# chernistry/sentio

Measured on NVIDIA B200. Metric: retrieval queries/sec @1M docs,1024-d,top_k=100, higher is better.
Workload: dtype f16 store / f32 scan / f64 exact re-score

## Files before the change

### sentio_b200/csrc/api.cu

```cuda
#include <stdarg.h>
#include <stdlib.h>

#include "common.cuh"

static thread_local char g_err[1024] = "";

void sb_set_error(const char* fmt, ...) {
  va_list ap;
  va_start(ap, fmt);
  vsnprintf(g_err, sizeof(g_err), fmt, ap);
  va_end(ap);
}

void ce_model_free(CeModel* m);
void ce_tokens_free(CeDocTokens* t);
void bm25_build_free(Bm25Build* b);

extern "C" {

const char* sb_last_error(void) { return g_err; }

int sb_version(void) { return 1000; }

int sb_create(int device, sb_ctx** out) {
  SB_REQUIRE(out != nullptr, SB_ERR_ARG, "sb_create: out is NULL");
  *out = nullptr;
  int ndev = 0;
  cudaError_t e = cudaGetDeviceCount(&ndev);
  if (e != cudaSuccess || ndev == 0) {
    sb_set_error("sb_create: no CUDA device visible (%s); libsentio_b200 has no CPU fallback",
                 e != cudaSuccess ? cudaGetErrorString(e) : "device count is 0");
    return SB_ERR_CUDA;
  }
  SB_REQUIRE(device >= 0 && device < ndev, SB_ERR_ARG, "sb_create: device %d out of range [0,%d)", device, ndev);
  DeviceGuard g(device);
  cudaDeviceProp prop;
  SB_CUDA(cudaGetDeviceProperties(&prop, device));
  SB_REQUIRE(prop.major == 10, SB_ERR_UNSUPPORTED,
             "sb_create: device %d is sm_%d%d; this library is built for sm_100a (B200) only", device, prop.major,
             prop.minor);
  sb_ctx* ctx = new sb_ctx();
  ctx->device = device;
  ctx->num_sms = prop.multiProcessorCount;
  ctx->smem_optin = prop.sharedMemPerBlockOptin;
  if (const char* v = getenv("SB_DENSE_PAIR")) ctx->dense_pair = atoi(v) != 0;
  if (const char* v = getenv("SB_DENSE_SAMPLE")) ctx->dense_sample_per_cta = atoi(v) > 0 ? atoi(v) : 2;
  if (const char* v = getenv("SB_DENSE_MULTISAMPLE")) ctx->dense_multisample = atoi(v) != 0;
  if (const char* v = getenv("SB_DENSE_PREFETCH")) ctx->dense_prefetch = atoi(v) > 0 ? atoi(v) : 0;
  if (const char* v = getenv("SB_DENSE_STAGES")) ctx->dense_max_stages = atoi(v) >= 3 ? atoi(v) : 8;
  cudaError_t se = cudaStreamCreateWithFlags(&ctx->stream, cudaStreamNonBlocking);
  if (se != cudaSuccess) {
    sb_set_error("sb_create: cudaStreamCreate failed: %s", cudaGetErrorString(se));
    delete ctx;
    return SB_ERR_CUDA;
  }
  *out = ctx;
  return SB_OK;
}

void sb_destroy(sb_ctx* ctx) {
  if (!ctx) return;
  DeviceGuard g(ctx->device);
  cudaStreamSynchronize(ctx->stream);
  for (int s = 0; s < SB_MAX_DENSE_SLOTS; ++s) {
    if (ctx->dense[s].rows) cudaFree(ctx->dense[s].rows);
    if (ctx->dense[s].inv_norm) cudaFree(ctx->dense[s].inv_norm);
  }
  Bm25Index& b = ctx->bm25;
  if (b.indptr) cudaFree(b.indptr);
  if (b.post_doc) cudaFree(b.post_doc);
  if (b.post_ratio) cudaFree(b.post_ratio);
  if (b.dnorm) cudaFree(b.dnorm);
  if (b.idf) cudaFree(b.idf);
  if (b.dense_of_term) cudaFree(b.dense_of_term);
  if (b.dense_ratio) cudaFree(b.dense_ratio);
  if (ctx->ce) ce_model_free(ctx->ce);
  if (ctx->enc) ce_model_free(ctx->enc);
  if (ctx->ce_tokens) ce_tokens_free(ctx->ce_tokens);
  if (ctx->bm25_build) bm25_build_free(ctx->bm25_build);
  ctx->q_dev.release();
  ctx->cand_dev.release();
  ctx->out_ids_dev.release();
  ctx->out_sc_dev.release();
  ctx->out_cnt_dev.release();
  ctx->misc_dev.release();
  ctx->misc2_dev.release();
  ctx->misc3_dev.release();
  ctx->acc_dev.release();
  ctx->qn_dev.release();
  ctx->qaux_dev.release();
  ctx->doc_chars_dev.release();
  ctx->pin_in.release();
  ctx->pin_out.release();
  ctx->hyb_pin.release();
  ctx->hyb_dev.release();
  for (auto& r : ctx->prof_recs) { cudaEventDestroy(r.a); cudaEventDestroy(r.b); }
  for (auto e : ctx->prof_pool) cudaEventDestroy(e);
  cudaStreamDestroy(ctx->stream);
// ... 67 lines not shown
```

### sentio_b200/csrc/common.cuh

```cuda
#pragma once
#include <cuda_runtime.h>
#include <cuda_fp16.h>
#include <stdint.h>
#include <stdio.h>
#include <mutex>
#include <string>
#include <vector>

#include "../../include/sentio_b200.h"

void sb_set_error(const char* fmt, ...);

#define SB_CUDA(expr)                                                                         \
  do {                                                                                        \
    cudaError_t _e = (expr);                                                                  \
    if (_e != cudaSuccess) {                                                                  \
      sb_set_error("CUDA error %s at %s:%d: %s", cudaGetErrorName(_e), __FILE__, __LINE__,    \
                   cudaGetErrorString(_e));                                                   \
      return SB_ERR_CUDA;                                                                     \
    }                                                                                         \
  } while (0)

#define SB_REQUIRE(cond, code, ...)  \
  do {                               \
// ... 51 lines not shown
    p = nullptr;
    cap = 0;
  }
  template <typename T>
  T* as() const { return reinterpret_cast<T*>(p); }
};

struct DenseIndex {
  int64_t n = 0;
  int64_t n_pad = 0;
  int32_t d = 0;
  int32_t d_pad = 0;
  int64_t id_base = 0;
  __half* rows = nullptr;
  float* inv_norm = nullptr;
  alignas(64) unsigned char tm_rows[128] = {0};
  const void* tm_rows_ptr = nullptr;
};

struct Bm25Index {
  int64_t n_docs = 0, n_terms = 0, nnz = 0;
  int64_t id_base = 0;
  int32_t variant = 0;
  double k1 = 1.5, b = 0.75, delta = 1.0, avgdl = 0.0;
  int64_t* indptr = nullptr;
  int32_t* post_doc = nullptr;
  double* post_ratio = nullptr;
  double* dnorm = nullptr;
  double* idf = nullptr;
  int32_t n_dense = 0;
  int32_t* dense_of_term = nullptr;
  double* dense_ratio = nullptr;
};

struct CeModel;
struct CeDocTokens;
struct Bm25Build;

struct sb_ctx {
  int device = 0;
  int num_sms = 0;
  size_t smem_optin = 0;
  cudaStream_t stream = nullptr;
  std::mutex mu;
  DenseIndex dense[SB_MAX_DENSE_SLOTS];
  Bm25Index bm25;
  CeModel* ce = nullptr;
  CeModel* enc = nullptr;
  CeDocTokens* ce_tokens = nullptr;
  Bm25Build* bm25_build = nullptr;
  int dense_mode = 0;
  int dense_pair = 1;
  int dense_sample_per_cta = 2;
  int max_clusters2 = 0;
  int dense_multisample = 1;
  int dense_prefetch = 0;
  int dense_max_stages = 8;
  uint64_t launches = 0;
  bool prof_on = false;
  struct ProfRec { int id; cudaEvent_t a, b; };
  std::vector<ProfRec> prof_recs;
  std::vector<cudaEvent_t> prof_pool;
  DevBuf q_dev, cand_dev, out_ids_dev, out_sc_dev, out_cnt_dev, misc_dev, misc2_dev, misc3_dev, acc_dev;
  DevBuf qn_dev;
  DevBuf qaux_dev;
  DevBuf doc_chars_dev;
  int64_t doc_chars_n = 0, doc_chars_base = 0;
  PinBuf pin_in, pin_out;
  std::mutex hyb_mu;
  PinBuf hyb_pin;
  DevBuf hyb_dev;
};

struct DeviceGuard {
  int prev = -1;
  explicit DeviceGuard(int dev) {
    cudaGetDevice(&prev);
    if (prev != dev) cudaSetDevice(dev);
  }
  ~DeviceGuard() {
    int cur = -1;
    cudaGetDevice(&cur);
    if (prev >= 0 && cur != prev) cudaSetDevice(prev);
  }
};

enum { SB_PROF_DENSE_SCAN = 0, SB_PROF_DENSE_MERGE = 1, SB_PROF_BM25_SCORE = 2, SB_PROF_BM25_SELECT = 3,
       SB_PROF_FUSE = 4, SB_PROF_CE = 5, SB_PROF_DENSE_SAMPLE = 6, SB_PROF_COUNT = 7 };

static inline cudaEvent_t prof_event(sb_ctx* ctx) {
  if (!ctx->prof_pool.empty()) {
    cudaEvent_t e = ctx->prof_pool.back();
    ctx->prof_pool.pop_back();
    return e;
  }
  cudaEvent_t e;
  cudaEventCreate(&e);
  return e;
}
struct ProfScope {
  sb_ctx* ctx;
  cudaStream_t st;
  cudaEvent_t b = nullptr;
  ProfScope(sb_ctx* c, int id, cudaStream_t s, int n_kernels = 1) : ctx(c), st(s) {
    ctx->launches += (uint64_t)n_kernels;
    if (ctx->prof_on) {
      cudaEvent_t a = prof_event(ctx);
// ... 152 lines not shown
```

### sentio_b200/csrc/dense_mma.cu

```cuda
#include <cuda.h>

#include <math.h>

#include <algorithm>
#include <vector>

#include "dense_common.cuh"
#include "dense_mma.cuh"

namespace {

constexpr int kTileRows = 128;
constexpr int kBK = 64;
constexpr uint32_t kATileBytes = kTileRows * kBK * 2;
constexpr int kMmaThreads = 192;
constexpr int kSelectThreads = 512;
constexpr int kSelStage = 8192;
constexpr int kSelTop = 2048;

__device__ __forceinline__ void tma_load_2d(uint32_t dst, const CUtensorMap* map, int c0, int c1, uint32_t bar) {
  asm volatile(
      "cp.async.bulk.tensor.2d.shared::cluster.global.mbarrier::complete_tx::bytes [%0], [%1, {%2, %3}], [%4];" ::"r"(dst),
      "l"(map), "r"(c0), "r"(c1), "r"(bar)
      : "memory");
// ... 4 lines not shown

__device__ __forceinline__ uint64_t make_smem_desc_sw128(uint32_t smem_addr) {
  uint64_t d = 0;
  d |= (uint64_t)((smem_addr >> 4) & 0x3fff);
  d |= (uint64_t)1 << 16;
  d |= (uint64_t)(1024 >> 4) << 32;
  d |= (uint64_t)1 << 46;
  d |= (uint64_t)2 << 61;
  return d;
}
__device__ __forceinline__ void umma_f16(uint32_t tmem_d, uint64_t a_desc, uint64_t b_desc, uint32_t idesc, uint32_t acc) {
  asm volatile(
      "{\n"
      ".reg .pred p;\n"
      "setp.ne.b32 p, %4, 0;\n"
      "tcgen05.mma.cta_group::1.kind::f16 [%0], %1, %2, %3, p;\n"
      "}\n" ::"r"(tmem_d),
      "l"(a_desc), "l"(b_desc), "r"(idesc), "r"(acc)
      : "memory");
}
__device__ __forceinline__ void umma_commit(uint32_t bar) {
  asm volatile("tcgen05.commit.cta_group::1.mbarrier::arrive::one.shared::cluster.b64 [%0];" ::"r"(bar) : "memory");
}

__device__ __forceinline__ uint32_t cluster_ctarank() {
  uint32_t r;
  asm volatile("mov.u32 %0, %%cluster_ctarank;" : "=r"(r));
  return r;
}
__device__ __forceinline__ uint32_t mapa_u32(uint32_t smem_addr, uint32_t rank) {
  uint32_t r;
  asm volatile("mapa.shared::cluster.u32 %0, %1, %2;" : "=r"(r) : "r"(smem_addr), "r"(rank));
  return r;
}
__device__ __forceinline__ void cluster_sync_all() {
  __syncwarp();
  asm volatile("barrier.cluster.arrive.release.aligned;\n\tbarrier.cluster.wait.acquire.aligned;" ::: "memory");
}
__device__ __forceinline__ void tma_load_2d_pair(uint32_t dst, const CUtensorMap* map, int c0, int c1, uint32_t bar_cluster) {
  asm volatile(
      "cp.async.bulk.tensor.2d.cta_group::2.shared::cluster.global.mbarrier::complete_tx::bytes [%0], [%1, {%2, %3}], [%4];" ::"r"(dst),
      "l"(map), "r"(c0), "r"(c1), "r"(bar_cluster)
      : "memory");
}
__device__ __forceinline__ void umma_f16_pair(uint32_t tmem_d, uint64_t a_desc, uint64_t b_desc, uint32_t idesc, uint32_t acc) {
  asm volatile(
      "{\n"
      ".reg .pred p;\n"
      "setp.ne.b32 p, %4, 0;\n"
      "tcgen05.mma.cta_group::2.kind::f16 [%0], %1, %2, %3, p;\n"
      "}\n" ::"r"(tmem_d),
      "l"(a_desc), "l"(b_desc), "r"(idesc), "r"(acc)
      : "memory");
}
__device__ __forceinline__ void umma_commit_pair(uint32_t bar) {
  asm volatile(
      "tcgen05.commit.cta_group::2.mbarrier::arrive::one.shared::cluster.multicast::cluster.b64 [%0], %1;" ::"r"(bar),
      "h"((uint16_t)3)
      : "memory");
}
__device__ __forceinline__ void mbar_arrive_cluster(uint32_t bar_cluster) {
  asm volatile("mbarrier.arrive.shared::cluster.b64 _, [%0];" ::"r"(bar_cluster) : "memory");
}

template <int N>
struct TmemLd;
template <>
struct TmemLd<16> {
  static __device__ __forceinline__ void ld(uint32_t taddr, uint32_t (&v)[16]) {
    asm volatile(
        "tcgen05.ld.sync.aligned.32x32b.x16.b32 {%0,%1,%2,%3,%4,%5,%6,%7,%8,%9,%10,%11,%12,%13,%14,%15}, [%16];"
        : "=r"(v[0]), "=r"(v[1]), "=r"(v[2]), "=r"(v[3]), "=r"(v[4]), "=r"(v[5]), "=r"(v[6]), "=r"(v[7]), "=r"(v[8]),
          "=r"(v[9]), "=r"(v[10]), "=r"(v[11]), "=r"(v[12]), "=r"(v[13]), "=r"(v[14]), "=r"(v[15])
        : "r"(taddr)
        : "memory");
  }
};

template <int NV>
__device__ __forceinline__ void sample_emit(const uint32_t (&v)[NV], bool live, float invn, unsigned long long* my_cand,
                                            size_t q_stride, int c0, int slot, int lane) {
#pragma unroll
  for (int j = 0; j < NV; ++j) {
    const float score = live ? __uint_as_float(v[j]) * invn : -INFINITY;
    const uint32_t best = __reduce_max_sync(0xffffffffu, f32_orderable(score));
    if (lane == (j & 31)) my_cand[(size_t)(c0 + j) * q_stride + slot] = ((unsigned long long)best << 32) | 0xffffffffull;
  }
}

struct MmaScanParams {
  const float* inv_norm;
  const float* thr_init;
  unsigned long long* cand;
  int32_t* counts;
  int32_t* fallback;
  int64_t n;
  int32_t kb_count;
  int32_t num_tiles;
  int32_t tile_first, tile_step;
  int32_t capg;
  int32_t stages;
  int32_t prefetch;
  int32_t n_groups;
  int64_t group_cand_stride;
  int64_t group_cnt_stride;
};

template <int QBN>
__global__ void __launch_bounds__(kMmaThreads, 1)
dense_scan_mma_kernel(const __grid_constant__ CUtensorMap tm_rows, const __grid_constant__ CUtensorMap tm_q,
                      const MmaScanParams p) {
  extern __shared__ uint8_t msm_raw[];
  const uint32_t raw = smem_u32(msm_raw);
  const uint32_t base = (raw + 1023u) & ~1023u;
  uint8_t* sm = msm_raw + (base - raw);
  constexpr uint32_t kQBlockBytes = QBN * kBK * 2;
  const uint32_t q_bytes = (uint32_t)p.kb_count * kQBlockBytes;
  const uint32_t a0 = base + q_bytes;
  uint64_t* bars = reinterpret_cast<uint64_t*>(sm + q_bytes + (size_t)p.stages * kATileBytes);
  const uint32_t bar_full = smem_u32(bars), bar_empty = smem_u32(bars + p.stages);
  const uint32_t bar_q = smem_u32(bars + 2 * p.stages);
  const uint32_t bar_acc_full = smem_u32(bars + 2 * p.stages + 1), bar_acc_empty = smem_u32(bars + 2 * p.stages + 3);
  uint32_t* tmem_slot = reinterpret_cast<uint32_t*>(bars + 2 * p.stages + 6);
  volatile float* thr = reinterpret_cast<volatile float*>(tmem_slot + 2);
  int* cnt = reinterpret_cast<int*>(const_cast<float*>(thr) + QBN);

  const int warp = threadIdx.x >> 5, lane = threadIdx.x & 31;
  const int grid = gridDim.x, cta = blockIdx.x;
  const int my_tiles = cta < p.num_tiles ? (p.num_tiles - 1 - cta) / grid + 1 : 0;

  if (threadIdx.x == 0) {
    for (int s = 0; s < p.stages; ++s) {
      mbar_init(bar_full + 8 * s, 1);
      mbar_init(bar_empty + 8 * s, 1);
    }
    mbar_init(bar_q, 1);
    for (int s = 0; s < 2; ++s) {
      mbar_init(bar_acc_full + 8 * s, 1);
      mbar_init(bar_acc_empty + 8 * s, 4);
    }
    mbar_fence_init();
    asm volatile("prefetch.tensormap [%0];" ::"l"(&tm_rows) : "memory");
    asm volatile("prefetch.tensormap [%0];" ::"l"(&tm_q) : "memory");
  }
  for (int i = threadIdx.x; i < QBN; i += blockDim.x) {
    thr[i] = p.thr_init ? p.thr_init[i] : -INFINITY;
    cnt[i] = 0;
  }
  if (warp == 1) {
    asm volatile("tcgen05.alloc.cta_group::1.sync.aligned.shared::cta.b32 [%0], %1;" ::"r"(smem_u32(tmem_slot)),
                 "n"(2 * QBN)
                 : "memory");
    asm volatile("tcgen05.relinquish_alloc_permit.cta_group::1.sync.aligned;" ::: "memory");
  }
// ... 48 lines not shown
        }
        umma_commit(bar_acc_full + 8 * as);
      }
    }
  } else {
    const int quad = warp & 3;
    unsigned long long* my_cand = p.cand + (size_t)cta * p.capg;
    const size_t q_stride = (size_t)grid * p.capg;
    for (int t = 0; t < my_tiles; ++t) {
      const int as = t & 1;
      const int tile = p.tile_first + (cta + t * grid) * p.tile_step;
      const int64_t row = (int64_t)tile * kTileRows + quad * 32 + lane;
      const float invn = row < p.n ? __ldg(p.inv_norm + row) : 0.f;
      mbar_wait(bar_acc_full + 8 * as, ((uint32_t)t >> 1) & 1u);
      asm volatile("tcgen05.fence::after_thread_sync;" ::: "memory");
#pragma unroll
      for (int c0 = 0; c0 < QBN; c0 += 16) {
        uint32_t v[16];
        TmemLd<16>::ld(tmem_base + ((uint32_t)(quad * 32) << 16) + (uint32_t)(as * QBN + c0), v);
        asm volatile("tcgen05.wait::ld.sync.aligned;" ::: "memory");
        if (p.thr_init == nullptr) {
          sample_emit<16>(v, row < p.n, invn, my_cand, q_stride, c0, t * 4 + quad, lane);
          continue;
        }
        if (row < p.n) {
#pragma unroll
          for (int j = 0; j < 16; ++j) {
            const float score = __uint_as_float(v[j]) * invn;
            if (score >= thr[c0 + j]) {
              const int pos = atomicAdd(&cnt[c0 + j], 1);
              if (pos < p.capg) my_cand[(size_t)(c0 + j) * q_stride + pos] = make_key32(score, (uint32_t)row);
            }
          }
        }
      }
      asm volatile("tcgen05.fence::before_thread_sync;" ::: "memory");
      __syncwarp();
      if (lane == 0) mbar_arrive(bar_acc_empty + 8 * as);
    }
  }
  asm volatile("tcgen05.fence::before_thread_sync;" ::: "memory");
  __syncthreads();
  for (int i = threadIdx.x; i < QBN; i += blockDim.x) {
    const int c = p.thr_init == nullptr ? my_tiles * 4 : cnt[i];
    p.counts[(size_t)i * grid + cta] = min(c, p.capg);
    if (c > p.capg && p.fallback) p.fallback[i] = 1;
  }
  if (warp == 1) {
    asm volatile("tcgen05.dealloc.cta_group::1.sync.aligned.b32 %0, %1;" ::"r"(tmem_base), "n"(2 * QBN) : "memory");
  }
}

template <int NQ>
__global__ void __cluster_dims__(2, 1, 1) __launch_bounds__(kMmaThreads, 1)
dense_scan_mma2_kernel(const __grid_constant__ CUtensorMap tm_rows, const __grid_constant__ CUtensorMap tm_q,
                       const MmaScanParams p) {
  constexpr int HQ = NQ / 2;
  extern __shared__ uint8_t msm_raw[];
  const uint32_t raw = smem_u32(msm_raw);
  const uint32_t base = (raw + 1023u) & ~1023u;
  uint8_t* sm = msm_raw + (base - raw);
  constexpr uint32_t kQBlockBytes = HQ * kBK * 2;
  const uint32_t q_bytes = (uint32_t)p.kb_count * kQBlockBytes;
  const uint32_t a0 = base + q_bytes;
  uint64_t* bars = reinterpret_cast<uint64_t*>(sm + q_bytes + (size_t)p.stages * kATileBytes);
  const uint32_t bar_full = smem_u32(bars), bar_empty = smem_u32(bars + p.stages);
  const uint32_t bar_q = smem_u32(bars + 2 * p.stages);
  const uint32_t bar_acc_full = smem_u32(bars + 2 * p.stages + 1), bar_acc_empty = smem_u32(bars + 2 * p.stages + 3);
  const uint32_t bar_qfree = smem_u32(bars + 2 * p.stages + 5);
  uint32_t* tmem_slot = reinterpret_cast<uint32_t*>(bars + 2 * p.stages + 8);
  volatile float* thr = reinterpret_cast<volatile float*>(tmem_slot + 2);
  int* cnt = reinterpret_cast<int*>(const_cast<float*>(thr) + NQ);

  const int warp = threadIdx.x >> 5, lane = threadIdx.x & 31;
  const uint32_t rank = cluster_ctarank();
  const int n_groups = p.thr_init == nullptr ? max(p.n_groups, 1) : 1;
  const int grid = gridDim.x, cta = blockIdx.x;
  const int pair = cta >> 1, npairs = grid >> 1;
  const int n_tp = (p.num_tiles + 1) >> 1;
  const int my_tiles = pair < n_tp ? (n_tp - 1 - pair) / npairs + 1 : 0;

  if (threadIdx.x == 0) {
    for (int s = 0; s < p.stages; ++s) {
      mbar_init(bar_full + 8 * s, 1);
      mbar_init(bar_empty + 8 * s, 1);
    }
    mbar_init(bar_q, 1);
    mbar_init(bar_qfree, 1);
    for (int s = 0; s < 2; ++s) {
      mbar_init(bar_acc_full + 8 * s, 1);
      mbar_init(bar_acc_empty + 8 * s, 8);
    }
    mbar_fence_init();
    asm volatile("prefetch.tensormap [%0];" ::"l"(&tm_rows) : "memory");
    asm volatile("prefetch.tensormap [%0];" ::"l"(&tm_q) : "memory");
  }
  for (int i = threadIdx.x; i < NQ; i += blockDim.x) {
    thr[i] = p.thr_init ? p.thr_init[i] : -INFINITY;
    cnt[i] = 0;
  }
  if (warp == 1) {
    asm volatile("tcgen05.alloc.cta_group::2.sync.aligned.shared::cta.b32 [%0], %1;" ::"r"(smem_u32(tmem_slot)),
                 "n"(2 * NQ)
                 : "memory");
    asm volatile("tcgen05.relinquish_alloc_permit.cta_group::2.sync.aligned;" ::: "memory");
  }
  asm volatile("tcgen05.fence::before_thread_sync;" ::: "memory");
  __syncthreads();
  cluster_sync_all();
  asm volatile("tcgen05.fence::after_thread_sync;" ::: "memory");
  const uint32_t tmem_base = *tmem_slot;

  if (warp == 0) {
    if (lane == 0) {
      const uint32_t lead_q = mapa_u32(bar_q, 0);
      int it = 0;
      const int total_it = my_tiles * p.kb_count;
      for (int g = 0; g < n_groups; ++g) {
      if (g > 0) mbar_wait(bar_qfree, (uint32_t)(g - 1) & 1u);
      if (rank == 0) mbar_expect_tx(bar_q, 2u * q_bytes);
      for (int kb = 0; kb < p.kb_count; ++kb)
        tma_load_2d_pair(base + (uint32_t)kb * kQBlockBytes, &tm_q, kb * kBK, g * NQ + (int)rank * HQ, lead_q);
      for (int t = 0; t < my_tiles; ++t) {
        const int li = 2 * (pair + t * npairs) + (int)rank;
        const int tile = li < p.num_tiles ? p.tile_first + li * p.tile_step : p.tile_first;
        for (int kb = 0; kb < p.kb_count; ++kb, ++it) {
          const int s = it % p.stages;
          const uint32_t use = (uint32_t)(it / p.stages);
          const int pf = (it - g * total_it) + p.stages + p.prefetch;
          if (p.prefetch > 0 && pf < total_it) {
            const int pt = pf / p.kb_count, pkb = pf - pt * p.kb_count;
            const int pli = 2 * (pair + pt * npairs) + (int)rank;
            if (pli < p.num_tiles) tma_prefetch_l2_2d(&tm_rows, pkb * kBK, (p.tile_first + pli * p.tile_step) * kTileRows);
          }
          if (it >= p.stages) mbar_wait(bar_empty + 8 * s, (use & 1u) ^ 1u);
          if (rank == 0) mbar_expect_tx(bar_full + 8 * s, 2u * kATileBytes);
          tma_load_2d_pair(a0 + (uint32_t)s * kATileBytes, &tm_rows, kb * kBK, tile * kTileRows,
                           mapa_u32(bar_full + 8 * s, 0));
        }
      }
      }
    }
  } else if (warp == 1) {
    if (lane == 0 && rank == 0) {
      const uint32_t idesc = (1u << 4) | ((uint32_t)(NQ >> 3) << 17) | ((uint32_t)(256 >> 4) << 24);
      int it = 0, tt = 0;
      for (int g = 0; g < n_groups; ++g) {
      mbar_wait(bar_q, (uint32_t)g & 1u);
      for (int t = 0; t < my_tiles; ++t, ++tt) {
        const int as = tt & 1;
        if (tt >= 2) mbar_wait(bar_acc_empty + 8 * as, (((uint32_t)tt >> 1) & 1u) ^ 1u);
        asm volatile("tcgen05.fence::after_thread_sync;" ::: "memory");
        const uint32_t d_tmem = tmem_base + (uint32_t)(as * NQ);
        for (int kb = 0; kb < p.kb_count; ++kb, ++it) {
          const int s = it % p.stages;
          const uint32_t use = (uint32_t)(it / p.stages);
          mbar_wait(bar_full + 8 * s, use & 1u);
          asm volatile("tcgen05.fence::after_thread_sync;" ::: "memory");
          const uint64_t da = make_smem_desc_sw128(a0 + (uint32_t)s * kATileBytes);
          const uint64_t db = make_smem_desc_sw128(base + (uint32_t)kb * kQBlockBytes);
#pragma unroll
          for (int k = 0; k < kBK / 16; ++k)
            umma_f16_pair(d_tmem, da + (uint64_t)(2 * k), db + (uint64_t)(2 * k), idesc, (kb | k) ? 1u : 0u);
          umma_commit_pair(bar_empty + 8 * s);
        }
        umma_commit_pair(bar_acc_full + 8 * as);
      }
      if (g + 1 < n_groups) umma_commit_pair(bar_qfree);
      }
    }
  } else {
    const int quad = warp & 3;
    const size_t q_stride = (size_t)grid * p.capg;
    int tt = 0;
    for (int g = 0; g < n_groups; ++g) {
    unsigned long long* my_cand = p.cand + (size_t)g * p.group_cand_stride + (size_t)cta * p.capg;
    for (int t = 0; t < my_tiles; ++t, ++tt) {
      const int as = tt & 1;
      const int li = 2 * (pair + t * npairs) + (int)rank;
      const int tile = p.tile_first + li * p.tile_step;
      const int64_t row = (int64_t)tile * kTileRows + quad * 32 + lane;
      const bool live = li < p.num_tiles && row < p.n;
      const float invn = live ? __ldg(p.inv_norm + row) : 0.f;
      mbar_wait(bar_acc_full + 8 * as, ((uint32_t)tt >> 1) & 1u);
      asm volatile("tcgen05.fence::after_thread_sync;" ::: "memory");
#pragma unroll 1
      for (int c0 = 0; c0 < NQ; c0 += 32) {
        uint32_t v[16], w[16];
        const uint32_t taddr = tmem_base + ((uint32_t)(quad * 32) << 16) + (uint32_t)(as * NQ + c0);
        TmemLd<16>::ld(taddr, v);
        TmemLd<16>::ld(taddr + 16u, w);
        asm volatile("tcgen05.wait::ld.sync.aligned;" ::: "memory");
        if (p.thr_init == nullptr) {
          sample_emit<16>(v, live, invn, my_cand, q_stride, c0, t * 4 + quad, lane);
          sample_emit<16>(w, live, invn, my_cand, q_stride, c0 + 16, t * 4 + quad, lane);
          continue;
        }
        if (live) {
#pragma unroll
          for (int j = 0; j < 32; ++j) {
            const float score = __uint_as_float(j < 16 ? v[j] : w[j - 16]) * invn;
            if (score >= thr[c0 + j]) {
              const int pos = atomicAdd(&cnt[c0 + j], 1);
              if (pos < p.capg) my_cand[(size_t)(c0 + j) * q_stride + pos] = make_key32(score, (uint32_t)row);
            }
          }
        }
      }
      asm volatile("tcgen05.fence::before_thread_sync;" ::: "memory");
      __syncwarp();
      if (lane == 0) mbar_arrive_cluster(mapa_u32(bar_acc_empty + 8 * as, 0));
    }
    }
  }
  asm volatile("tcgen05.fence::before_thread_sync;" ::: "memory");
  __syncthreads();
  for (int i = threadIdx.x; i < NQ * n_groups; i += blockDim.x) {
    const int g = i / NQ, qi = i - g * NQ;
    const int c = p.thr_init == nullptr ? my_tiles * 4 : cnt[qi];
    p.counts[(size_t)g * p.group_cnt_stride + (size_t)qi * grid + cta] = min(c, p.capg);
    if (c > p.capg && p.fallback) p.fallback[qi] = 1;
// ... 145 lines not shown
  ra.k = p.k;
  ra.out_ids = p.out_ids + (size_t)qi * p.k;
  ra.out_scores = p.out_scores + (size_t)qi * p.k;
  ra.out_count = p.out_counts + qi;
  rescore_and_emit(top, ntop, P, ek, ei, &qq_s, reinterpret_cast<float*>(keys), ra);
}

typedef CUresult (*EncodeTiledFn)(CUtensorMap*, CUtensorMapDataType, cuuint32_t, void*, const cuuint64_t*,
                                  const cuuint64_t*, const cuuint32_t*, const cuuint32_t*, CUtensorMapInterleave,
                                  CUtensorMapSwizzle, CUtensorMapL2promotion, CUtensorMapFloatOOBfill);

int encode_map(CUtensorMap* map, const void* ptr, int64_t rows, int64_t cols, int box_rows) {
  static EncodeTiledFn fn = nullptr;
  if (!fn) {
    void* pfn = nullptr;
    cudaDriverEntryPointQueryResult qres;
    if (cudaGetDriverEntryPoint("cuTensorMapEncodeTiled", &pfn, cudaEnableDefault, &qres) == cudaSuccess &&
        qres == cudaDriverEntryPointSuccess)
      fn = reinterpret_cast<EncodeTiledFn>(pfn);
  }
  SB_REQUIRE(fn != nullptr, SB_ERR_CUDA, "cuTensorMapEncodeTiled entry point not available");
  cuuint64_t dims[2] = {(cuuint64_t)cols, (cuuint64_t)rows};
  cuuint64_t strides[1] = {(cuuint64_t)cols * 2};
  cuuint32_t box[2] = {(cuuint32_t)kBK, (cuuint32_t)box_rows};
  cuuint32_t estr[2] = {1, 1};
  CUresult r = fn(map, CU_TENSOR_MAP_DATA_TYPE_FLOAT16, 2, const_cast<void*>(ptr), dims, strides, box, estr,
                  CU_TENSOR_MAP_INTERLEAVE_NONE, CU_TENSOR_MAP_SWIZZLE_128B, CU_TENSOR_MAP_L2_PROMOTION_L2_256B,
                  CU_TENSOR_MAP_FLOAT_OOB_FILL_NONE);
  SB_REQUIRE(r == CUDA_SUCCESS, SB_ERR_CUDA, "cuTensorMapEncodeTiled failed with CUresult %d", (int)r);
  return SB_OK;
}

template <int QBN>
int launch_mma(const CUtensorMap& tm_rows, const CUtensorMap& tm_q, const MmaScanParams& mp, int grid, size_t smem,
               cudaStream_t st) {
  auto kern = dense_scan_mma_kernel<QBN>;
  SB_CUDA(cudaFuncSetAttribute(kern, cudaFuncAttributeMaxDynamicSharedMemorySize, (int)smem));
  kern<<<grid, kMmaThreads, smem, st>>>(tm_rows, tm_q, mp);
  SB_CUDA(cudaGetLastError());
  return SB_OK;
}

int dispatch_mma(int qbn, const CUtensorMap& tm_rows, const CUtensorMap& tm_q, const MmaScanParams& mp, int grid,
                 size_t smem, cudaStream_t st) {
  switch (qbn) {
    case 16: return launch_mma<16>(tm_rows, tm_q, mp, grid, smem, st);
    case 32: return launch_mma<32>(tm_rows, tm_q, mp, grid, smem, st);
    case 64: return launch_mma<64>(tm_rows, tm_q, mp, grid, smem, st);
  }
  sb_set_error("dense_mma: unsupported query block %d", qbn);
  return SB_ERR_UNSUPPORTED;
}

int launch_mma_pair(const CUtensorMap& tm_rows, const CUtensorMap& tm_q, const MmaScanParams& mp, int grid, size_t smem,
                    cudaStream_t st) {
  auto kern = dense_scan_mma2_kernel<128>;
  SB_CUDA(cudaFuncSetAttribute(kern, cudaFuncAttributeMaxDynamicSharedMemorySize, (int)smem));
  kern<<<grid, kMmaThreads, smem, st>>>(tm_rows, tm_q, mp);
  SB_CUDA(cudaGetLastError());
  return SB_OK;
}

int pair_clusters(sb_ctx* ctx, size_t smem) {
  if (ctx->max_clusters2 > 0) return ctx->max_clusters2;
  auto kern = dense_scan_mma2_kernel<128>;
  int n = 0;
  if (cudaFuncSetAttribute(kern, cudaFuncAttributeMaxDynamicSharedMemorySize, (int)smem) == cudaSuccess) {
    cudaLaunchConfig_t cfg = {};
    cfg.gridDim = dim3((unsigned)(ctx->num_sms & ~1), 1, 1);
    cfg.blockDim = dim3(kMmaThreads, 1, 1);
    cfg.dynamicSmemBytes = smem;
    cudaLaunchAttribute at[1];
    at[0].id = cudaLaunchAttributeClusterDimension;
    at[0].val.clusterDim.x = 2;
    at[0].val.clusterDim.y = 1;
    at[0].val.clusterDim.z = 1;
    cfg.attrs = at;
    cfg.numAttrs = 1;
    if (cudaOccupancyMaxActiveClusters(&n, kern, &cfg) != cudaSuccess) n = 0;
  }
  (void)cudaGetLastError();
  if (n <= 0 || n > ctx->num_sms / 2) n = ctx->num_sms / 2;
  ctx->max_clusters2 = n;
  return n;
}

}

bool dense_mma_eligible(const sb_ctx* ctx, const DenseIndex& ix, int B) {
  if (B < 16) return false;
  if (ix.d_pad % kBK != 0 || ix.n_pad % kTileRows != 0) return false;
  if (ix.n < 64 * kTileRows) return false;
  const size_t need = (size_t)ix.d_pad * 16 * 2 + 3 * (size_t)kATileBytes + 4096;
  return need <= ctx->smem_optin;
}

int dense_mma_topk_enqueue(sb_ctx* ctx, DenseIndex& ix, const float* q_pad, int B, int k, int64_t* out_ids,
                           double* out_scores, int32_t* out_counts, cudaStream_t st) {
  const int kb_count = ix.d_pad / kBK;
  const int total_tiles = (int)(ix.n_pad / kTileRows);
  int qbn_max = 64;
  while (qbn_max > 16 && (size_t)qbn_max * ix.d_pad * 2 + 3 * (size_t)kATileBytes + 4096 > ctx->smem_optin) qbn_max >>= 1;
  const bool pair_ok = ctx->dense_pair != 0 && qbn_max == 64 && total_tiles >= 2;
  const int gsz = pair_ok ? 128 : qbn_max;
  const int grid1 = std::min(ctx->num_sms, total_tiles);
  int grid2 = 0, stages2 = 0;
  size_t smem2 = 0;
  if (pair_ok) {
    const size_t q_bytes = (size_t)64 * ix.d_pad * 2;
    stages2 = std::max(3, std::min((int)((ctx->smem_optin - q_bytes - 3072) / kATileBytes), ctx->dense_max_stages));
    smem2 = q_bytes + (size_t)stages2 * kATileBytes + 2048 + 1024;
    grid2 = 2 * std::min(pair_clusters(ctx, smem2), (total_tiles + 1) / 2);
  }
  const int grid = std::max(grid1, grid2);
  const int grid_min = grid2 > 0 ? std::min(grid1, grid2) : grid1;
  const int per_cta = std::max(ctx->dense_sample_per_cta, std::min(8, (k + grid - 1) / grid));
  const int sample_tiles = std::min(per_cta * grid, total_tiles);
  const int sample_step = total_tiles / sample_tiles;
  const int sgrid1 = std::min(grid1, sample_tiles);
  const int sgrid2 = pair_ok ? std::min(grid2, (sample_tiles + 1) & ~1) : 0;
  const int sgrid = std::max(sgrid1, sgrid2);
  const int sgrid_min = sgrid2 > 0 ? std::min(sgrid1, sgrid2) : sgrid1;
  const int64_t worst = (int64_t)((total_tiles + grid_min - 1) / grid_min + 1) * kTileRows;
  const int64_t samp_keys = (int64_t)((sample_tiles + sgrid_min - 1) / sgrid_min + 1) * 4;
  const double f = (double)k / (4.0 * sample_tiles);
  const double pass = f >= 0.95 ? 1.0 : -log(1.0 - f) / 32.0;
  const int64_t expect = (int64_t)((double)worst * pass) + 1;
  const int capg = (int)std::min<int64_t>(worst, std::max<int64_t>(8 * expect + 256, samp_keys));
  int rc;
  SB_REQUIRE(grid <= kSelectThreads, SB_ERR_UNSUPPORTED, "dense_mma: %d CTAs exceed the select kernel's prefix width", grid);
  const int n_groups = (B + gsz - 1) / gsz;
  const size_t cand_per_group = (size_t)gsz * grid * capg * 8;
  int gmax = (int)std::max<size_t>(1, (size_t)(1024ull << 20) / cand_per_group);
  gmax = std::min(gmax, n_groups);
  if ((rc = ctx->misc2_dev.reserve((size_t)n_groups * gsz * ix.d_pad * 2 + 256))) return rc;
  if ((rc = ctx->misc3_dev.reserve(((size_t)gsz * 4 + (size_t)gsz * grid * 4) * gmax + 256))) return rc;
  if ((rc = ctx->cand_dev.reserve(cand_per_group * gmax))) return rc;
  __half* q16 = ctx->misc2_dev.as<__half>();
  float* thr = ctx->misc3_dev.as<float>();
  int32_t* counts = reinterpret_cast<int32_t*>(thr + (size_t)gsz * gmax);
  unsigned long long* cand = ctx->cand_dev.as<unsigned long long>();
  if (ix.tm_rows_ptr != ix.rows) {
    if ((rc = encode_map(reinterpret_cast<CUtensorMap*>(ix.tm_rows), ix.rows, ix.n_pad, ix.d_pad, kTileRows))) return rc;
    ix.tm_rows_ptr = ix.rows;
  }
  const CUtensorMap& tm_rows = *reinterpret_cast<const CUtensorMap*>(ix.tm_rows);
  const size_t sel_smem = (size_t)kSelStage * 8 + (size_t)kSelTop * 20 + 64;
  SB_CUDA(cudaFuncSetAttribute(dense_select_kernel, cudaFuncAttributeMaxDynamicSharedMemorySize, (int)sel_smem));
  float* eps = nullptr;
  int32_t* fb = nullptr;
  if ((rc = dense_prep_queries(ctx, ix, q_pad, B, n_groups * gsz, true, nullptr, q16, &eps, &fb, st))) return rc;

  for (int c0 = 0; c0 < B; c0 += gmax * gsz) {
    const int nq_chunk = std::min(B - c0, gmax * gsz);
    const int ng = (nq_chunk + gsz - 1) / gsz;
    struct Group { int qbn, nq; bool pair; CUtensorMap tm_q; size_t smem; int stages; };
    std::vector<Group> gs((size_t)ng);
    int rows_total = 0;
    for (int g = 0; g < ng; ++g) {
      Group& G = gs[(size_t)g];
      const int left = nq_chunk - g * gsz;
      __half* q16g = q16 + (size_t)(c0 + g * gsz) * ix.d_pad;
      G.pair = pair_ok && left > 64;
      if (G.pair) {
        G.qbn = 128;
        G.nq = std::min(128, left);
        if ((rc = encode_map(&G.tm_q, q16g, 128, ix.d_pad, 64))) return rc;
        G.stages = stages2;
        G.smem = smem2;
      } else {
        G.qbn = qbn_max;
        while (G.qbn > 16 && G.qbn / 2 >= left) G.qbn >>= 1;
        G.nq = std::min(G.qbn, left);
        if ((rc = encode_map(&G.tm_q, q16g, G.qbn, ix.d_pad, G.qbn))) return rc;
        const size_t q_bytes = (size_t)G.qbn * ix.d_pad * 2;
        G.stages = std::max(3, std::min((int)((ctx->smem_optin - q_bytes - 3072) / kATileBytes), ctx->dense_max_stages));
        G.smem = q_bytes + (size_t)G.stages * kATileBytes + 2048 + 1024;
      }
      rows_total = g * gsz + G.qbn;
    }
    MmaScanParams mp;
    mp.inv_norm = ix.inv_norm;
    mp.n = ix.n;
    mp.kb_count = kb_count;
    mp.capg = capg;
    mp.prefetch = ctx->dense_prefetch;
    mp.n_groups = 1;
    mp.group_cand_stride = 0;
    mp.group_cnt_stride = 0;
    SelectParams sp;
    sp.cand = cand;
    sp.counts = counts;
    sp.capg = capg;
    sp.nq = nq_chunk;
    sp.thr_out = thr;
    sp.eps = eps + c0;
    sp.fallback = fb + c0;
    sp.rows = ix.rows;
    sp.q = q_pad + (size_t)c0 * ix.d_pad;
    sp.d_pad = ix.d_pad;
    sp.ch = ix.d_pad / 8;
    sp.id_base = ix.id_base;
    sp.k = k;
    sp.out_ids = out_ids + (size_t)c0 * k;
    sp.out_scores = out_scores + (size_t)c0 * k;
    sp.out_counts = out_counts + c0;
    mp.thr_init = nullptr;
    mp.fallback = nullptr;
    mp.num_tiles = sample_tiles;
    mp.tile_first = 0;
    mp.tile_step = sample_step;
    {
      ProfScope ps(ctx, SB_PROF_DENSE_SAMPLE, st, ng + 1);
      int g_first = 0;
      int n_pair = 0;
      while (n_pair < ng && gs[(size_t)n_pair].pair) ++n_pair;
      if (ctx->dense_multisample != 0 && n_pair >= 2) {
        CUtensorMap tm_q_all;
        if ((rc = encode_map(&tm_q_all, q16 + (size_t)c0 * ix.d_pad, (int64_t)n_pair * 128, ix.d_pad, 64))) return rc;
        mp.cand = cand;
        mp.counts = counts;
        mp.stages = stages2;
        mp.n_groups = n_pair;
        mp.group_cand_stride = (int64_t)gsz * sgrid * capg;
        mp.group_cnt_stride = (int64_t)gsz * sgrid;
        if ((rc = launch_mma_pair(tm_rows, tm_q_all, mp, sgrid, smem2, st))) return rc;
        mp.n_groups = 1;
        g_first = n_pair;
      }
      for (int g = g_first; g < ng; ++g) {
        const Group& G = gs[(size_t)g];
        mp.cand = cand + (size_t)g * gsz * sgrid * capg;
        mp.counts = counts + (size_t)g * gsz * sgrid;
        mp.stages = G.stages;
        if (G.pair) rc = launch_mma_pair(tm_rows, G.tm_q, mp, sgrid, G.smem, st);
        else rc = dispatch_mma(G.qbn, tm_rows, G.tm_q, mp, sgrid, G.smem, st);
        if (rc) return rc;
      }
      sp.grid = sgrid;
      sp.mode = 0;
      dense_select_kernel<<<rows_total, kSelectThreads, sel_smem, st>>>(sp);
    }
    SB_CUDA(cudaGetLastError());
    mp.num_tiles = total_tiles;
    mp.tile_first = 0;
    mp.tile_step = 1;
    for (int g = 0; g < ng; ++g) {
      const Group& G = gs[(size_t)g];
      mp.thr_init = thr + (size_t)g * gsz;
      mp.fallback = fb + c0 + (size_t)g * gsz;
      mp.cand = cand + (size_t)g * gsz * grid * capg;
      mp.counts = counts + (size_t)g * gsz * grid;
      mp.stages = G.stages;
      ProfScope ps(ctx, SB_PROF_DENSE_SCAN, st);
      if (G.pair) rc = launch_mma_pair(tm_rows, G.tm_q, mp, grid, G.smem, st);
      else rc = dispatch_mma(G.qbn, tm_rows, G.tm_q, mp, grid, G.smem, st);
      if (rc) return rc;
    }
    sp.grid = grid;
    sp.mode = 1;
    {
      ProfScope ps(ctx, SB_PROF_DENSE_MERGE, st);
      dense_select_kernel<<<nq_chunk, kSelectThreads, sel_smem, st>>>(sp);
    }
    SB_CUDA(cudaGetLastError());
  }
  return dense_fallback_enqueue(ctx, ix, q_pad, B, k, fb, out_ids, out_scores, out_counts, st);
}
```

Before: 251,200.

## Add wide 256-query cluster-pair scan kernel with streamed query tiles

Adds a 256-query variant of the 2-CTA cluster MMA scan, enabled by default when the batch exceeds 128 queries. Each streamed document tile is then reused across twice as many queries, roughly halving document-matrix traffic per query. Query blocks no longer fit resident in shared memory, so an extra producer warp streams them through a small ring with their own barriers. L2 cache hints mark document rows evict-first and query tiles evict-last. The cost is more query reloads from L2, an extra warp and barrier traffic, and fewer document pipeline stages.

New measurement: 296,800 (median of 6 runs). 1.18x the previous value.

```diff
diff --git a/sentio_b200/csrc/api.cu b/sentio_b200/csrc/api.cu
--- a/sentio_b200/csrc/api.cu
+++ b/sentio_b200/csrc/api.cu
@@ -44,6 +44,8 @@
   ctx->num_sms = prop.multiProcessorCount;
   ctx->smem_optin = prop.sharedMemPerBlockOptin;
   if (const char* v = getenv("SB_DENSE_PAIR")) ctx->dense_pair = atoi(v) != 0;
+  if (const char* v = getenv("SB_DENSE_WIDE")) ctx->dense_wide = atoi(v) != 0;
+  if (const char* v = getenv("SB_DENSE_QSTAGES")) ctx->dense_q_stages = atoi(v) >= 2 ? atoi(v) : 4;
   if (const char* v = getenv("SB_DENSE_SAMPLE")) ctx->dense_sample_per_cta = atoi(v) > 0 ? atoi(v) : 2;
   if (const char* v = getenv("SB_DENSE_MULTISAMPLE")) ctx->dense_multisample = atoi(v) != 0;
   if (const char* v = getenv("SB_DENSE_PREFETCH")) ctx->dense_prefetch = atoi(v) > 0 ? atoi(v) : 0;
diff --git a/sentio_b200/csrc/common.cuh b/sentio_b200/csrc/common.cuh
--- a/sentio_b200/csrc/common.cuh
+++ b/sentio_b200/csrc/common.cuh
@@ -127,7 +127,10 @@
   int dense_mode = 0;
   int dense_pair = 1;
   int dense_sample_per_cta = 2;
+  int dense_wide = 1;
+  int dense_q_stages = 4;
   int max_clusters2 = 0;
+  int max_clusters2w = 0;
   int dense_multisample = 1;
   int dense_prefetch = 0;
   int dense_max_stages = 8;
diff --git a/sentio_b200/csrc/dense_mma.cu b/sentio_b200/csrc/dense_mma.cu
--- a/sentio_b200/csrc/dense_mma.cu
+++ b/sentio_b200/csrc/dense_mma.cu
@@ -80,6 +80,23 @@
       "}\n" ::"r"(tmem_d),
       "l"(a_desc), "l"(b_desc), "r"(idesc), "r"(acc)
       : "memory");
+}
+__device__ __forceinline__ void tma_load_2d_pair_hint(uint32_t dst, const CUtensorMap* map, int c0, int c1,
+                                                      uint32_t bar_cluster, uint64_t policy) {
+  asm volatile(
+      "cp.async.bulk.tensor.2d.cta_group::2.shared::cluster.global.mbarrier::complete_tx::bytes.L2::cache_hint [%0], [%1, {%2, %3}], [%4], %5;" ::"r"(dst),
+      "l"(map), "r"(c0), "r"(c1), "r"(bar_cluster), "l"(policy)
+      : "memory");
+}
+__device__ __forceinline__ uint64_t l2_policy_evict_first() {
+  uint64_t pol;
+  asm volatile("createpolicy.fractional.L2::evict_first.b64 %0, 1.0;" : "=l"(pol));
+  return pol;
+}
+__device__ __forceinline__ uint64_t l2_policy_evict_last() {
+  uint64_t pol;
+  asm volatile("createpolicy.fractional.L2::evict_last.b64 %0, 1.0;" : "=l"(pol));
+  return pol;
 }
 __device__ __forceinline__ void umma_commit_pair(uint32_t bar) {
   asm volatile(
@@ -128,6 +145,7 @@
   int32_t tile_first, tile_step;
   int32_t capg;
   int32_t stages;
+  int32_t q_stages;
   int32_t prefetch;
   int32_t n_groups;
   int64_t group_cand_stride;
@@ -282,23 +300,30 @@
 }
 
 template <int NQ>
-__global__ void __cluster_dims__(2, 1, 1) __launch_bounds__(kMmaThreads, 1)
+constexpr int pair_threads() { return NQ > 128 ? kMmaThreads + 32 : kMmaThreads; }
+
+template <int NQ>
+__global__ void __cluster_dims__(2, 1, 1) __launch_bounds__(pair_threads<NQ>(), 1)
 dense_scan_mma2_kernel(const __grid_constant__ CUtensorMap tm_rows, const __grid_constant__ CUtensorMap tm_q,
                        const MmaScanParams p) {
+  constexpr bool kStreamQ = NQ > 128;
   constexpr int HQ = NQ / 2;
   extern __shared__ uint8_t msm_raw[];
   const uint32_t raw = smem_u32(msm_raw);
   const uint32_t base = (raw + 1023u) & ~1023u;
   uint8_t* sm = msm_raw + (base - raw);
   constexpr uint32_t kQBlockBytes = HQ * kBK * 2;
-  const uint32_t q_bytes = (uint32_t)p.kb_count * kQBlockBytes;
+  const int q_stages = kStreamQ ? p.q_stages : 0;
+  const uint32_t q_bytes = (uint32_t)(kStreamQ ? p.q_stages : p.kb_count) * kQBlockBytes;
   const uint32_t a0 = base + q_bytes;
   uint64_t* bars = reinterpret_cast<uint64_t*>(sm + q_bytes + (size_t)p.stages * kATileBytes);
   const uint32_t bar_full = smem_u32(bars), bar_empty = smem_u32(bars + p.stages);
   const uint32_t bar_q = smem_u32(bars + 2 * p.stages);
   const uint32_t bar_acc_full = smem_u32(bars + 2 * p.stages + 1), bar_acc_empty = smem_u32(bars + 2 * p.stages + 3);
   const uint32_t bar_qfree = smem_u32(bars + 2 * p.stages + 5);
-  uint32_t* tmem_slot = reinterpret_cast<uint32_t*>(bars + 2 * p.stages + 8);
+  const uint32_t bar_qfull = smem_u32(bars + 2 * p.stages + 6);
+  const uint32_t bar_qempty = smem_u32(bars + 2 * p.stages + 6 + q_stages);
+  uint32_t* tmem_slot = reinterpret_cast<uint32_t*>(bars + 2 * p.stages + 8 + 2 * q_stages);
   volatile float* thr = reinterpret_cast<volatile float*>(tmem_slot + 2);
   int* cnt = reinterpret_cast<int*>(const_cast<float*>(thr) + NQ);
 
@@ -317,6 +342,10 @@
     }
     mbar_init(bar_q, 1);
     mbar_init(bar_qfree, 1);
+    for (int s = 0; s < q_stages; ++s) {
+      mbar_init(bar_qfull + 8 * s, 1);
+      mbar_init(bar_qempty + 8 * s, 1);
+    }
     for (int s = 0; s < 2; ++s) {
       mbar_init(bar_acc_full + 8 * s, 1);
       mbar_init(bar_acc_empty + 8 * s, 8);
@@ -344,13 +373,16 @@
   if (warp == 0) {
     if (lane == 0) {
       const uint32_t lead_q = mapa_u32(bar_q, 0);
+      const uint64_t pol_rows = kStreamQ ? l2_policy_evict_first() : 0ull;
       int it = 0;
       const int total_it = my_tiles * p.kb_count;
       for (int g = 0; g < n_groups; ++g) {
-      if (g > 0) mbar_wait(bar_qfree, (uint32_t)(g - 1) & 1u);
-      if (rank == 0) mbar_expect_tx(bar_q, 2u * q_bytes);
-      for (int kb = 0; kb < p.kb_count; ++kb)
-        tma_load_2d_pair(base + (uint32_t)kb * kQBlockBytes, &tm_q, kb * kBK, g * NQ + (int)rank * HQ, lead_q);
+      if constexpr (!kStreamQ) {
+        if (g > 0) mbar_wait(bar_qfree, (uint32_t)(g - 1) & 1u);
+        if (rank == 0) mbar_expect_tx(bar_q, 2u * q_bytes);
+        for (int kb = 0; kb < p.kb_count; ++kb)
+          tma_load_2d_pair(base + (uint32_t)kb * kQBlockBytes, &tm_q, kb * kBK, g * NQ + (int)rank * HQ, lead_q);
+      }
       for (int t = 0; t < my_tiles; ++t) {
         const int li = 2 * (pair + t * npairs) + (int)rank;
         const int tile = li < p.num_tiles ? p.tile_first + li * p.tile_step : p.tile_first;
@@ -365,18 +397,37 @@
           }
           if (it >= p.stages) mbar_wait(bar_empty + 8 * s, (use & 1u) ^ 1u);
           if (rank == 0) mbar_expect_tx(bar_full + 8 * s, 2u * kATileBytes);
-          tma_load_2d_pair(a0 + (uint32_t)s * kATileBytes, &tm_rows, kb * kBK, tile * kTileRows,
-                           mapa_u32(bar_full + 8 * s, 0));
+          if constexpr (kStreamQ)
+            tma_load_2d_pair_hint(a0 + (uint32_t)s * kATileBytes, &tm_rows, kb * kBK, tile * kTileRows,
+                                  mapa_u32(bar_full + 8 * s, 0), pol_rows);
+          else
+            tma_load_2d_pair(a0 + (uint32_t)s * kATileBytes, &tm_rows, kb * kBK, tile * kTileRows,
+                             mapa_u32(bar_full + 8 * s, 0));
         }
       }
       }
+    }
+  } else if (warp == kMmaThreads / 32) {
+    if constexpr (kStreamQ) if (lane == 0) {
+      const uint64_t pol_q = l2_policy_evict_last();
+      int it = 0;
+      for (int g = 0; g < n_groups; ++g)
+        for (int t = 0; t < my_tiles; ++t)
+          for (int kb = 0; kb < p.kb_count; ++kb, ++it) {
+            const int s = it % q_stages;
+            const uint32_t use = (uint32_t)(it / q_stages);
+            if (it >= q_stages) mbar_wait(bar_qempty + 8 * s, (use & 1u) ^ 1u);
+            if (rank == 0) mbar_expect_tx(bar_qfull + 8 * s, 2u * kQBlockBytes);
+            tma_load_2d_pair_hint(base + (uint32_t)s * kQBlockBytes, &tm_q, kb * kBK, g * NQ + (int)rank * HQ,
+                                  mapa_u32(bar_qfull + 8 * s, 0), pol_q);
+          }
     }
   } else if (warp == 1) {
     if (lane == 0 && rank == 0) {
       const uint32_t idesc = (1u << 4) | ((uint32_t)(NQ >> 3) << 17) | ((uint32_t)(256 >> 4) << 24);
       int it = 0, tt = 0;
       for (int g = 0; g < n_groups; ++g) {
-      mbar_wait(bar_q, (uint32_t)g & 1u);
+      if constexpr (!kStreamQ) mbar_wait(bar_q, (uint32_t)g & 1u);
       for (int t = 0; t < my_tiles; ++t, ++tt) {
         const int as = tt & 1;
         if (tt >= 2) mbar_wait(bar_acc_empty + 8 * as, (((uint32_t)tt >> 1) & 1u) ^ 1u);
@@ -386,17 +437,23 @@
           const int s = it % p.stages;
           const uint32_t use = (uint32_t)(it / p.stages);
           mbar_wait(bar_full + 8 * s, use & 1u);
+          int qs = kb;
+          if constexpr (kStreamQ) {
+            qs = it % q_stages;
+            mbar_wait(bar_qfull + 8 * qs, (uint32_t)(it / q_stages) & 1u);
+          }
           asm volatile("tcgen05.fence::after_thread_sync;" ::: "memory");
           const uint64_t da = make_smem_desc_sw128(a0 + (uint32_t)s * kATileBytes);
-          const uint64_t db = make_smem_desc_sw128(base + (uint32_t)kb * kQBlockBytes);
+          const uint64_t db = make_smem_desc_sw128(base + (uint32_t)qs * kQBlockBytes);
 #pragma unroll
           for (int k = 0; k < kBK / 16; ++k)
             umma_f16_pair(d_tmem, da + (uint64_t)(2 * k), db + (uint64_t)(2 * k), idesc, (kb | k) ? 1u : 0u);
           umma_commit_pair(bar_empty + 8 * s);
+          if constexpr (kStreamQ) umma_commit_pair(bar_qempty + 8 * qs);
         }
         umma_commit_pair(bar_acc_full + 8 * as);
       }
-      if (g + 1 < n_groups) umma_commit_pair(bar_qfree);
+      if (!kStreamQ && g + 1 < n_groups) umma_commit_pair(bar_qfree);
       }
     }
   } else {
@@ -648,23 +705,34 @@
   return SB_ERR_UNSUPPORTED;
 }
 
+template <int NQ>
 int launch_mma_pair(const CUtensorMap& tm_rows, const CUtensorMap& tm_q, const MmaScanParams& mp, int grid, size_t smem,
                     cudaStream_t st) {
-  auto kern = dense_scan_mma2_kernel<128>;
+  auto kern = dense_scan_mma2_kernel<NQ>;
   SB_CUDA(cudaFuncSetAttribute(kern, cudaFuncAttributeMaxDynamicSharedMemorySize, (int)smem));
-  kern<<<grid, kMmaThreads, smem, st>>>(tm_rows, tm_q, mp);
+  kern<<<grid, pair_threads<NQ>(), smem, st>>>(tm_rows, tm_q, mp);
   SB_CUDA(cudaGetLastError());
   return SB_OK;
 }
 
-int pair_clusters(sb_ctx* ctx, size_t smem) {
-  if (ctx->max_clusters2 > 0) return ctx->max_clusters2;
-  auto kern = dense_scan_mma2_kernel<128>;
+enum GroupKind { kSingle, kPair, kWide };
+
+int launch_group(GroupKind kind, int qbn, const CUtensorMap& tm_rows, const CUtensorMap& tm_q, const MmaScanParams& mp,
+                 int grid, size_t smem, cudaStream_t st) {
+  if (kind == kWide) return launch_mma_pair<256>(tm_rows, tm_q, mp, grid, smem, st);
+  if (kind == kPair) return launch_mma_pair<128>(tm_rows, tm_q, mp, grid, smem, st);
+  return dispatch_mma(qbn, tm_rows, tm_q, mp, grid, smem, st);
+}
+
+template <int NQ>
+int pair_clusters(sb_ctx* ctx, size_t smem, int& cache) {
+  if (cache > 0) return cache;
+  auto kern = dense_scan_mma2_kernel<NQ>;
   int n = 0;
   if (cudaFuncSetAttribute(kern, cudaFuncAttributeMaxDynamicSharedMemorySize, (int)smem) == cudaSuccess) {
     cudaLaunchConfig_t cfg = {};
     cfg.gridDim = dim3((unsigned)(ctx->num_sms & ~1), 1, 1);
-    cfg.blockDim = dim3(kMmaThreads, 1, 1);
+    cfg.blockDim = dim3(pair_threads<NQ>(), 1, 1);
     cfg.dynamicSmemBytes = smem;
     cudaLaunchAttribute at[1];
     at[0].id = cudaLaunchAttributeClusterDimension;
@@ -677,7 +745,7 @@
   }
   (void)cudaGetLastError();
   if (n <= 0 || n > ctx->num_sms / 2) n = ctx->num_sms / 2;
-  ctx->max_clusters2 = n;
+  cache = n;
   return n;
 }
 
@@ -698,25 +766,40 @@
   int qbn_max = 64;
   while (qbn_max > 16 && (size_t)qbn_max * ix.d_pad * 2 + 3 * (size_t)kATileBytes + 4096 > ctx->smem_optin) qbn_max >>= 1;
   const bool pair_ok = ctx->dense_pair != 0 && qbn_max == 64 && total_tiles >= 2;
-  const int gsz = pair_ok ? 128 : qbn_max;
+  const bool wide = ctx->dense_wide != 0 && B > 128 && total_tiles >= 2;
+  const int gsz = wide ? 256 : pair_ok ? 128 : qbn_max;
   const int grid1 = std::min(ctx->num_sms, total_tiles);
   int grid2 = 0, stages2 = 0;
   size_t smem2 = 0;
   if (pair_ok) {
     const size_t q_bytes = (size_t)64 * ix.d_pad * 2;
     stages2 = std::max(3, std::min((int)((ctx->smem_optin - q_bytes - 3072) / kATileBytes), ctx->dense_max_stages));
-    smem2 = q_bytes + (size_t)stages2 * kATileBytes + 2048 + 1024;
-    grid2 = 2 * std::min(pair_clusters(ctx, smem2), (total_tiles + 1) / 2);
-  }
-  const int grid = std::max(grid1, grid2);
-  const int grid_min = grid2 > 0 ? std::min(grid1, grid2) : grid1;
+    smem2 = q_bytes + (size_t)stages2 * kATileBytes + 2048 + 128 * 8;
+    grid2 = 2 * std::min(pair_clusters<128>(ctx, smem2, ctx->max_clusters2), (total_tiles + 1) / 2);
+  }
+  int gridw = 0, stagesw = 0, qstagesw = 0;
+  size_t smemw = 0;
+  if (wide) {
+    qstagesw = ctx->dense_q_stages;
+    const size_t q_bytes = (size_t)qstagesw * kATileBytes;
+    stagesw = std::max(3, std::min((int)((ctx->smem_optin - q_bytes - 2048 - 256 * 8) / kATileBytes), ctx->dense_max_stages));
+    smemw = q_bytes + (size_t)stagesw * kATileBytes + 2048 + 256 * 8;
+    gridw = 2 * std::min(pair_clusters<256>(ctx, smemw, ctx->max_clusters2w), (total_tiles + 1) / 2);
+  }
+  const int grid = std::max(grid1, std::max(grid2, gridw));
+  int grid_min = grid1;
+  if (grid2 > 0) grid_min = std::min(grid_min, grid2);
+  if (gridw > 0) grid_min = std::min(grid_min, gridw);
   const int per_cta = std::max(ctx->dense_sample_per_cta, std::min(8, (k + grid - 1) / grid));
   const int sample_tiles = std::min(per_cta * grid, total_tiles);
   const int sample_step = total_tiles / sample_tiles;
   const int sgrid1 = std::min(grid1, sample_tiles);
   const int sgrid2 = pair_ok ? std::min(grid2, (sample_tiles + 1) & ~1) : 0;
-  const int sgrid = std::max(sgrid1, sgrid2);
-  const int sgrid_min = sgrid2 > 0 ? std::min(sgrid1, sgrid2) : sgrid1;
+  const int sgridw = wide ? std::min(gridw, (sample_tiles + 1) & ~1) : 0;
+  const int sgrid = std::max(sgrid1, std::max(sgrid2, sgridw));
+  int sgrid_min = sgrid1;
+  if (sgrid2 > 0) sgrid_min = std::min(sgrid_min, sgrid2);
+  if (sgridw > 0) sgrid_min = std::min(sgrid_min, sgridw);
   const int64_t worst = (int64_t)((total_tiles + grid_min - 1) / grid_min + 1) * kTileRows;
   const int64_t samp_keys = (int64_t)((sample_tiles + sgrid_min - 1) / sgrid_min + 1) * 4;
   const double f = (double)k / (4.0 * sample_tiles);
@@ -749,37 +832,39 @@
 
   for (int c0 = 0; c0 < B; c0 += gmax * gsz) {
     const int nq_chunk = std::min(B - c0, gmax * gsz);
-    const int ng = (nq_chunk + gsz - 1) / gsz;
-    struct Group { int qbn, nq; bool pair; CUtensorMap tm_q; size_t smem; int stages; };
-    std::vector<Group> gs((size_t)ng);
+    struct Group { int off, qbn, nq; GroupKind kind; CUtensorMap tm_q; size_t smem; int stages; };
+    std::vector<Group> gs;
     int rows_total = 0;
-    for (int g = 0; g < ng; ++g) {
-      Group& G = gs[(size_t)g];
-      const int left = nq_chunk - g * gsz;
-      __half* q16g = q16 + (size_t)(c0 + g * gsz) * ix.d_pad;
-      G.pair = pair_ok && left > 64;
-      if (G.pair) {
-        G.qbn = 128;
-        G.nq = std::min(128, left);
-        if ((rc = encode_map(&G.tm_q, q16g, 128, ix.d_pad, 64))) return rc;
-        G.stages = stages2;
-        G.smem = smem2;
+    while (rows_total < nq_chunk) {
+      Group G;
+      G.off = rows_total;
+      const int left = nq_chunk - G.off;
+      __half* q16g = q16 + (size_t)(c0 + G.off) * ix.d_pad;
+      G.kind = wide && left > 128 ? kWide : pair_ok && left > 64 ? kPair : kSingle;
+      if (G.kind != kSingle) {
+        G.qbn = G.kind == kWide ? 256 : 128;
+        if ((rc = encode_map(&G.tm_q, q16g, G.qbn, ix.d_pad, G.qbn / 2))) return rc;
+        G.stages = G.kind == kWide ? stagesw : stages2;
+        G.smem = G.kind == kWide ? smemw : smem2;
       } else {
         G.qbn = qbn_max;
         while (G.qbn > 16 && G.qbn / 2 >= left) G.qbn >>= 1;
-        G.nq = std::min(G.qbn, left);
         if ((rc = encode_map(&G.tm_q, q16g, G.qbn, ix.d_pad, G.qbn))) return rc;
         const size_t q_bytes = (size_t)G.qbn * ix.d_pad * 2;
         G.stages = std::max(3, std::min((int)((ctx->smem_optin - q_bytes - 3072) / kATileBytes), ctx->dense_max_stages));
         G.smem = q_bytes + (size_t)G.stages * kATileBytes + 2048 + 1024;
       }
-      rows_total = g * gsz + G.qbn;
-    }
+      G.nq = std::min(G.qbn, left);
+      rows_total += G.qbn;
+      gs.push_back(G);
+    }
+    const int ng = (int)gs.size();
     MmaScanParams mp;
     mp.inv_norm = ix.inv_norm;
     mp.n = ix.n;
     mp.kb_count = kb_count;
     mp.capg = capg;
+    mp.q_stages = qstagesw;
     mp.prefetch = ctx->dense_prefetch;
     mp.n_groups = 1;
     mp.group_cand_stride = 0;
@@ -809,29 +894,28 @@
     {
       ProfScope ps(ctx, SB_PROF_DENSE_SAMPLE, st, ng + 1);
       int g_first = 0;
-      int n_pair = 0;
-      while (n_pair < ng && gs[(size_t)n_pair].pair) ++n_pair;
-      if (ctx->dense_multisample != 0 && n_pair >= 2) {
+      int n_lead = 0;
+      while (gs[0].kind != kSingle && n_lead < ng && gs[(size_t)n_lead].kind == gs[0].kind) ++n_lead;
+      if (ctx->dense_multisample != 0 && n_lead >= 2) {
+        const Group& G = gs[0];
         CUtensorMap tm_q_all;
-        if ((rc = encode_map(&tm_q_all, q16 + (size_t)c0 * ix.d_pad, (int64_t)n_pair * 128, ix.d_pad, 64))) return rc;
+        if ((rc = encode_map(&tm_q_all, q16 + (size_t)c0 * ix.d_pad, (int64_t)n_lead * G.qbn, ix.d_pad, G.qbn / 2))) return rc;
         mp.cand = cand;
         mp.counts = counts;
-        mp.stages = stages2;
-        mp.n_groups = n_pair;
-        mp.group_cand_stride = (int64_t)gsz * sgrid * capg;
-        mp.group_cnt_stride = (int64_t)gsz * sgrid;
-        if ((rc = launch_mma_pair(tm_rows, tm_q_all, mp, sgrid, smem2, st))) return rc;
+        mp.stages = G.stages;
+        mp.n_groups = n_lead;
+        mp.group_cand_stride = (int64_t)G.qbn * sgrid * capg;
+        mp.group_cnt_stride = (int64_t)G.qbn * sgrid;
+        if ((rc = launch_group(G.kind, G.qbn, tm_rows, tm_q_all, mp, sgrid, G.smem, st))) return rc;
         mp.n_groups = 1;
-        g_first = n_pair;
+        g_first = n_lead;
       }
       for (int g = g_first; g < ng; ++g) {
         const Group& G = gs[(size_t)g];
-        mp.cand = cand + (size_t)g * gsz * sgrid * capg;
-        mp.counts = counts + (size_t)g * gsz * sgrid;
+        mp.cand = cand + (size_t)G.off * sgrid * capg;
+        mp.counts = counts + (size_t)G.off * sgrid;
         mp.stages = G.stages;
-        if (G.pair) rc = launch_mma_pair(tm_rows, G.tm_q, mp, sgrid, G.smem, st);
-        else rc = dispatch_mma(G.qbn, tm_rows, G.tm_q, mp, sgrid, G.smem, st);
-        if (rc) return rc;
+        if ((rc = launch_group(G.kind, G.qbn, tm_rows, G.tm_q, mp, sgrid, G.smem, st))) return rc;
       }
       sp.grid = sgrid;
       sp.mode = 0;
@@ -843,15 +927,13 @@
     mp.tile_step = 1;
     for (int g = 0; g < ng; ++g) {
       const Group& G = gs[(size_t)g];
-      mp.thr_init = thr + (size_t)g * gsz;
-      mp.fallback = fb + c0 + (size_t)g * gsz;
-      mp.cand = cand + (size_t)g * gsz * grid * capg;
-      mp.counts = counts + (size_t)g * gsz * grid;
+      mp.thr_init = thr + (size_t)G.off;
+      mp.fallback = fb + c0 + (size_t)G.off;
+      mp.cand = cand + (size_t)G.off * grid * capg;
+      mp.counts = counts + (size_t)G.off * grid;
       mp.stages = G.stages;
       ProfScope ps(ctx, SB_PROF_DENSE_SCAN, st);
-      if (G.pair) rc = launch_mma_pair(tm_rows, G.tm_q, mp, grid, G.smem, st);
-      else rc = dispatch_mma(G.qbn, tm_rows, G.tm_q, mp, grid, G.smem, st);
-      if (rc) return rc;
+      if ((rc = launch_group(G.kind, G.qbn, tm_rows, G.tm_q, mp, grid, G.smem, st))) return rc;
     }
     sp.grid = grid;
     sp.mode = 1;
```
